# Denizantip/py-numpy-renderer

Measured on AMD Instinct MI355X. Metric: Mfrag/s (1920x1080, 200k tris + shadow volumes), higher is better.
Workload: dtype f64; 1 GPU; torus 500x200 (200k tris) + floor, 1920x1080, point light, shadow volumes (BASELINE.json configs[3] / BASELINE.md c4); faces=200002, views=8, frames_in_flight=3, parallelism=screen tiles x1 (bands)

## Files before the change

### py-numpy-renderer_amd/csrc/host_env.h

```cpp
#pragma once

namespace {

struct Env {
    bool vertex_mfma, resolve_separate, sil_cache, big_tri_reject;
    int edge_spread, tile_split, tile_order;
    int quad_walk;
    int pair_log;
    int ao_shape, dof_shape, mblur_shape, taa_shape;
    int bloom_shape;
    int tone_form, tone_grid;
    unsigned split_cost, split_quads;
    const char *cluster_cull;
};

Env read_env()
{
    static const Env once = [] {
        auto is = [](const char *name, const char *value) { const char *e = getenv(name); return e && !strcmp(e, value); };
        auto number = [](const char *name, int unset) { const char *e = getenv(name); return e ? atoi(e) : unset; };
        auto shape = [&](const char *name, const char *s0, const char *s1, const char *s2) {
            return is(name, s0) ? 0 : is(name, s1) ? 1 : is(name, s2) ? 2 : 0;
        };
        Env e = {};
// ... 9 lines not shown
        e.ao_shape = shape("MR_AO_TILE", "64x64", "32x32", "64x16");
        e.dof_shape = shape("MR_DOF_TILE", "32x32", "32x32x256", "16x16");
        e.mblur_shape = shape("MR_MBLUR_TILE", "32x32", "32x32x256", "16x16");
        e.taa_shape = shape("MR_TAA_TILE", "32x8", "64x4", "16x16");
        e.bloom_shape = shape("MR_BLOOM_TILE", "32x8", "64x4", "16x16");
        e.tone_form = is("MR_TONEMAP_HIST", "ballot") ? 1 : 0;
        e.tone_grid = std::min(std::max(number("MR_TONEMAP_GRID", (int)mr::TONE_HIST_BLOCKS), 1), (int)mr::TONE_MAX_BLOCKS);
        return e;
    }();
    Env e = once;
    e.cluster_cull = getenv("MR_CLUSTER_CULL");
    const char *sil = getenv("MR_SIL_CACHE");
    e.sil_cache = !(sil && !strcmp(sil, "0"));
    const char *rej = getenv("MR_BIG_TRI_REJECT");
    e.big_tri_reject = !(rej && !strcmp(rej, "0"));
    return e;
}

}
```

### py-numpy-renderer_amd/csrc/host_frame.h

```cpp
#pragma once

namespace {

constexpr int EVENT_RING = 512, N_MARKS = 6;

struct FrameSlot {
    hipStream_t stream = nullptr;
    int id = 0;
    DevBuf d_vout, d_vclip, d_tris, d_clips, d_status, d_count_list, d_quads, d_sil, d_counters;
    DevBuf d_bin_count, d_items[mr::BIN_CLASSES], d_work, d_tile_stats, d_hist, d_split;
    DevBuf d_z, d_winner, d_stencil, d_frame, d_out;
    DevBuf d_frame_b;
    DevBuf d_bloom;
    DevBuf d_shafts;
    DevBuf d_tone;
    int last_tone = 0;
    float last_tone_exposure = 0.f;
    MotionSlot motion;
    MotionFacesSlot motion_faces;
    LayersSlot layers;
    int last_layers = 0;
    bool last_motion = false;
    DevBuf d_stencil_x[mr::MAX_LIGHTS - 1];
    static_assert(mr::MAX_LIGHTS == MR_MAX_LIGHTS, "the ABI's light count is the kernels'");
    int last_n_lights = 1;
// ... 12 lines not shown

    mr_frame_desc last_frame = {};
    int last_n_tiles = 0;
    bool last_ordered = false;
    bool last_full = false, last_split = false;
    bool overlay_deferred = false;
    int last_ss_mode = 0;
    bool last_post = false;
    bool have_frame = false, stats_reduced = false;
    bool last_copied = false;

    void reset_caps() { bins_zeroed_for = 0; have_frame = false; }
    void release()
    {
        for (DevBuf *b : { &d_vout, &d_vclip, &d_count_list, &d_tris, &d_clips, &d_status, &d_quads, &d_sil, &d_counters,
                           &d_bin_count, &d_work, &d_tile_stats, &d_hist, &d_split, &d_z, &d_winner, &d_stencil, &d_frame, &d_frame_b, &d_bloom, &d_shafts, &d_tone, &d_out })
            b->release();
        for (DevBuf &b : d_items) b.release();
        for (DevBuf &b : d_stencil_x) b.release();
        motion.release();
        motion_faces.release();
        layers.release();
        ov.release();
        if (events_ok) {
            for (auto &set : ev_ring) for (auto &e : set) (void)hipEventDestroy(e);
            (void)hipHostFree(h_counters);
            events_ok = false;
        }
    }
    mr::Counters *ctr(uint64_t frame) const { return d_counters.as<mr::Counters>() + (frame & 1); }
    mr::Sticky *sticky() const { return reinterpret_cast<mr::Sticky *>(d_counters.as<mr::Counters>() + 2); }
// ... 335 lines not shown
        { fs->d_frame_b, p.dof || p.motion || p.taa ? kept_f * 3 * sizeof(float) : 0 },
        { fs->d_bloom, p.bloom ? bloom_pyramid(fc.width, fc.height, p.bloom_params.levels).floats * sizeof(float) : 0 },
        { fs->d_shafts, p.shafts ? 2 * shafts_level(fc.width, fc.height, p.shafts_params.levels).device_floats() * sizeof(float) : 0 },
        { fs->d_tone, p.tone ? tone_slot_bytes(tone_grid(fc.width, fc.height, p.env)) : 0 } };
    for (const auto &b : sized) HIP_TRY(b.buf.ensure(b.bytes));
    if (p.taa)
        if (int rc = grow_history(sc, fc.width, fc.height)) return rc;
    for (int k = 1; k < p.n_lights; ++k) HIP_TRY(fs->d_stencil_x[k - 1].ensure(kept * sizeof(int32_t)));
    if (int rc = ensure_cleared(fs->d_counters, 2 * sizeof(Counters) + sizeof(Sticky), fs->stream)) return rc;
    for (int c = 0; c < BIN_CLASSES; ++c) {
        const size_t bytes = nT * fs->bin_cap[c] * 4;
        if (bytes > ((size_t)48 << 30))
            return fail(MR_E_OVERFLOW, "more primitives in one 16x16 tile than the tile lists are allowed to grow to (48 GB per class)");
        HIP_TRY(fs->d_items[c].ensure(bytes));
    }
    if (!fs->events_ok) {
        for (auto &set : fs->ev_ring) for (auto &e : set) HIP_TRY(hipEventCreate(&e));
        HIP_TRY(hipHostMalloc((void **)&fs->h_counters, sizeof(Counters) + sizeof(Sticky), hipHostMallocDefault));
        fs->h_sticky = reinterpret_cast<Sticky *>(fs->h_counters + 1);
        fs->events_ok = true;
    }
    return MR_OK;
}

int grow_tile_state(FrameSlot *fs, const FramePlan &p)
{
    using namespace mr;
    HIP_TRY(fs->d_hist.ensure(p.order_bytes + (size_t)std::max(p.n_tiles, 1) + 16));
    constexpr size_t arrive_bytes = (size_t)HEAVY0_MAX * 4;
    if (int rc = ensure_cleared(fs->d_split, arrive_bytes + arrive_bytes * HEAVY_SPLIT * TILE_PX, fs->stream, arrive_bytes)) return rc;
    if (fs->bins_zeroed_for != BIN_CLASSES * p.n_tiles + 1) {
        HIP_TRY(hipMemsetAsync(fs->d_bin_count.p, 0, fs->d_bin_count.cap, fs->stream));
        HIP_TRY(hipMemsetAsync(fs->d_hist.p, 0, fs->d_hist.cap, fs->stream));
        fs->bins_zeroed_for = BIN_CLASSES * p.n_tiles + 1;
    }
    return MR_OK;
}

mr::BinArgs bin_args(const FrameSlot *fs)
{
    mr::BinArgs ba;
    ba.tris = fs->d_tris.as<mr::TriRec>(); ba.quads = fs->d_quads.as<mr::QuadRec>();
    ba.ctr = fs->ctr(fs->frames_enqueued); ba.quad_cap = fs->quad_cap;
    ba.bin_count = fs->d_bin_count.as<uint32_t>();
    for (int c = 0; c < mr::BIN_CLASSES; ++c) { ba.items[c] = fs->d_items[c].as<uint32_t>(); ba.cap[c] = fs->bin_cap[c]; }
    ba.work = fs->d_work.as<uint2>(); ba.work_cap = fs->work_cap;
    return ba;
}

int launch_setup(mr_scene *sc, FrameSlot *fs, const mr::FrameConst &fc, const FramePlan &p, const mr::FrameLights &lights)
{
    using namespace mr;
    hipStream_t stream = fs->stream;
    SetupKernArgs ska;
    ska.fc = fc; ska.bins = bin_args(fs); ska.face_blocks = p.face_blocks;
    SetupArgs &sa = ska.sa;
    sa.faces = sc->d_faces.as<int32_t>(); sa.face_flags = sc->d_face_flags.as<uint8_t>();
    sa.verts = sc->d_verts.as<double>(); sa.uv = sc->d_uv.as<float>(); sa.normals = sc->d_normals.as<float>();
    sa.vout = fs->d_vout.as<VertexOut>(); sa.vclip = fs->d_vclip.as<VertexClip>();
    sa.face_pos = sc->d_face_pos.p; sa.clusters = sc->d_clusters.as<ClusterRec>();
    sa.tris = fs->d_tris.as<TriRec>(); sa.clips = fs->d_clips.as<TriClip>();
// ... 40 lines not shown
    TileArgs &ta = tka.ta;
    ta.clips = fs->d_clips.as<TriClip>(); ta.quads = fs->d_quads.as<QuadRec>();
    ta.bin_count = fs->d_bin_count.as<uint32_t>();
    for (int c = 0; c < BIN_CLASSES; ++c) { ta.items[c] = fs->d_items[c].as<uint32_t>(); ta.cap[c] = fs->bin_cap[c]; }
    ta.tap_mask = (p.overlay && !p.taps_asked) ? fs->ov.list<uint8_t>(3) : nullptr;
    ta.zbuf = p.keep ? fs->d_z.as<double>() : nullptr;
    ta.winner = p.keep ? fs->d_winner.as<int32_t>() : nullptr;
    ta.stencil = p.keep ? fs->d_stencil.as<int32_t>() : nullptr;
    ta.tile_stats = fs->d_tile_stats.as<uint32_t>();
    ta.ctr = fs->ctr(fs->frames_enqueued); ta.next_ctr = fs->ctr(fs->frames_enqueued + 1); ta.sticky = fs->sticky();
    ta.order = p.ordered ? fs->d_hist.as<uint32_t>() : nullptr;
    ta.tile_class = reinterpret_cast<uint8_t *>(fs->d_hist.p) + p.order_bytes;
    ta.split_arrive = fs->d_split.as<uint32_t>(); ta.split_sten = fs->d_split.as<int32_t>() + HEAVY0_MAX;
    ta.split_cost = p.split_cost; ta.split_quads = p.split_quads; ta.split_max = p.split_max;
    ta.quad_walk = (uint32_t)p.env.quad_walk;
    ta.pair_log = (uint32_t)fc.n_faces <= PAIR_LOG_MAX_FACE ? (uint32_t)p.env.pair_log : 0u;
    ShadeArgs &sh = tka.sh;
    sh.tris = fs->d_tris.as<TriRec>(); sh.face_pos = sc->d_face_pos.p; sh.face_attr = sc->d_face_attr.as<FaceAttr>();
    sh.materials = sc->d_materials.as<Material>();
    sh.sky = sc->sky_size > 0 ? sc->d_sky.as<uint8_t>() : nullptr;
    sh.gamma_lut = sc->d_gamma.as<float>(); sh.out = d_out;
    sh.frame = (fc.flags & MR_FRAME_KEEP_FLOAT) ? fs->d_frame.as<float>() : nullptr;
    tka.ml.lights.n = 1;
    if (p.ml) tka.ml.lights = lights;
    for (int k = 1; p.ml && k < MAX_LIGHTS; ++k) tka.ml.stencil[k - 1] = p.keep && k < p.n_lights ? fs->d_stencil_x[k - 1].as<int32_t>() : nullptr;
    if (p.n_tiles <= 0) {
        HIP_TRY(hipMemsetAsync(ta.next_ctr, 0, sizeof(Counters), fs->stream));
        return MR_OK;
    }
    static const struct { void (*kernel)(const TileKernArgs); int front; } choice[2][6] = {
// ... 225 lines not shown
```

### py-numpy-renderer_amd/csrc/kernels_bin.h

```cpp
#pragma once

#include "rast_math.h"
#include "tri_reject.h"

namespace mr {

struct TileSpan { int tx0, tx1, ty0, ty1; };

__device__ __forceinline__ int tile_row_frame(const FrameConst &fc, int l) { return fc.tile_y0 + l * fc.tile_step; }

__device__ __forceinline__ bool tile_span(const FrameConst &fc, int x0, int x1, int y0, int y1, TileSpan &s)
{
    y0 = max(y0, fc.band_y0);
    y1 = min(y1, fc.band_y1);
    if (x0 >= x1 || y0 >= y1) return false;
    s.tx0 = x0 / TILE_W;            s.tx1 = (x1 - 1) / TILE_W + 1;
    const int g0 = y0 / TILE_H - fc.tile_y0, g1 = (y1 - 1) / TILE_H - fc.tile_y0;
    if (g1 < 0) return false;
    const int st = fc.tile_step;
    s.ty0 = g0 <= 0 ? 0 : (g0 + st - 1) / st;
    s.ty1 = min(g1 / st + 1, fc.tiles_y);
    return s.ty0 < s.ty1;
}

// ... 14 lines not shown
    bool out = o0 || o1 || o2 || (n > 3 && o3);
    for (int i = 4; i < n && !out; ++i) out = outside(q.e[i]);
    return !out;
}

struct BinArgs {
    const TriRec *tris;
    const QuadRec *quads;
    Counters *ctr;
    uint32_t quad_cap;
    uint32_t *bin_count;
    uint32_t *items[BIN_CLASSES];
    uint32_t cap[BIN_CLASSES];
    uint2 *work;
    uint32_t work_cap;
};

constexpr int TILE_STATS = 5;
constexpr int TILE_REC = 12;
constexpr int QUAD_BATCH = 64;
constexpr int BIN_SMALL = 4;
constexpr uint32_t WORK_QUAD = 0x80000000u;
constexpr int ORDER_CLASSES = 8;
constexpr int ORDER_HEAD = 4;

struct PrimBox { int x0, x1, y0, y1; };

__device__ __forceinline__ int pair_class(const FrameConst &fc, bool is_quad, bool clip, const PrimBox &pb, int tx, int ty)
{
    if (is_quad) return 2;
// ... 156 lines not shown
        if (!tile_span(fc, pb.x0, pb.x1, pb.y0, pb.y1, sp)) continue;
        const int bw = sp.tx1 - sp.tx0, total = bw * (sp.ty1 - sp.ty0);
        const int j = (int)item.y * WAVE + lane;
        if (j >= total) continue;
        const int tx = sp.tx0 + j % bw, ty = sp.ty0 + j / bw;
        bool touches;
        if (is_quad) {
            touches = quad_touches_tile(a.quads[id], tx, tile_row_frame(fc, ty));
        } else {
            touches = !big_tri_reject || tri_touches_tile(a.tris[id], tx * TILE_W, tile_row_frame(fc, ty) * TILE_H);
            if (fc.flags & MR_FRAME_COUNTERS) {
                const unsigned long long out = __ballot(!touches);
                if (out && lane == __ffsll((long long)out) - 1) atomicAdd(&a.ctr->pad0[7], (unsigned int)__popcll(out));
            }
        }
        if (touches) bin_emit(fc, a, pair_class(fc, is_quad, clip, pb, tx, ty), id, tx, ty);
    }
}

__device__ void order_tiles_block(const uint8_t *__restrict__ cls, uint32_t *__restrict__ order, int n_tiles)
{
    constexpr int NT = 256, NW = NT / WAVE, NC = ORDER_CLASSES + 1, FIELD = 12, LOW = 5;
    __shared__ uint32_t s_cnt[NC][NT];
    __shared__ uint32_t s_tot[NC];
    const int tid = threadIdx.x, lane = tid & (WAVE - 1), wv = tid / WAVE;
    const int per = ((n_tiles + NT - 1) / NT + 3) & ~3;
    const int t0 = tid * per, nwords = per >> 2;
    const uint32_t *__restrict__ words = reinterpret_cast<const uint32_t *>(cls);
    auto fetch = [&](int i) -> uint32_t {
        const int t = t0 + 4 * i;
        uint32_t v = t < n_tiles ? words[t >> 2] : 0xffffffffu;
// ... 76 lines not shown
```

### py-numpy-renderer_amd/csrc/kernels_tile.h

```cpp
#pragma once

#include "kernels_bin.h"
#include "kernels_shade.h"
#include "rast_resolve.h"

namespace mr {

__device__ __forceinline__ unsigned long long z_key(double z)
{
    const unsigned long long b = (unsigned long long)__double_as_longlong(z);
    return (b >> 63) ? ~b : (b | 0x8000000000000000ull);
}
__device__ __forceinline__ double z_unkey(unsigned long long k)
{
    const unsigned long long b = (k >> 63) ? (k & 0x7fffffffffffffffull) : ~k;
    return __longlong_as_double((long long)b);
}

template <bool MAYBE_SINGLE>
struct PairMath {
    double a0, a1, p0, p1, q0, q1, k0, k1, k2;
    float d00, d01, d11, inv_den;
    bool sbox, sz;
    __device__ __forceinline__ explicit PairMath(const TriRec &t)
// ... 132 lines not shown
    double nx, ny, nz, d;
    int16_t x0, x1, y0, y1;
    int32_t n, is_front, edge;
    uint32_t pad[3];
};
static_assert(sizeof(QuadHead) == 64, "QuadHead mirrors QuadRec's header");

enum : uint32_t { QUAD_WALK_AUTO = 0, QUAD_WALK_STRIPS = 1, QUAD_WALK_SPANS = 2 };
#ifndef MR_SPAN_MIN_EDGES
#define MR_SPAN_MIN_EDGES 1
#endif
#ifndef MR_SPAN_MIN_QUADS
#define MR_SPAN_MIN_QUADS 6
#endif

__device__ __forceinline__ bool quad_depth_pass(double q_nx, double q_ny, double nzq, double q_d, double a0, double b0,
                                                double dpx, double dpy, double zbest, bool rh, bool in,
                                                double f_plus_n, double f_minus_n, double two_nf)
{
    const double t = (q_nx * dpx + q_ny * dpy) + q_d;
    const double tf = t * f_minus_n;
    const double den = a0 + tf;
    const double prod = zbest * den;
    const double e = prod - b0;
    const bool zinf = fabs(zbest) == INFINITY;
    bool pass = zinf ? (rh ? zbest > 0 : zbest < 0) : (rh ? ((e > 0) == (den > 0)) : ((e < 0) == (den > 0)));
    const bool clear = zinf || fabs(e) > 1e-9 * (fabs(prod) + fabs(b0));
    const bool unsure = in && !(clear && fabs(den) > 2e-4 * (fabs(a0) + fabs(tf)));
    if (__ballot(unsure)) {
        if (unsure) {
            const double z = two_nf / (f_plus_n - (-t / nzq) * f_minus_n);
            pass = rh ? (zbest >= z) : (zbest <= z);
        }
    }
    return pass;
}

constexpr int MAT_LDS = 8;
static_assert(sizeof(Material) % 8 == 0 && MAT_LDS * sizeof(Material) / 8 <= TILE_PX, "material staging");

#ifndef MR_CLASS_SCALE
#define MR_CLASS_SCALE 100
#endif
__device__ __forceinline__ int tile_class(uint32_t cost)
{
    const uint32_t c = cost * 100u / (uint32_t)MR_CLASS_SCALE;
    return c >= 500u ? 1 : c >= 350u ? 2 : c >= 250u ? 3 : c >= 170u ? 4 : c >= 110u ? 5 : c >= 70u ? 6 : c >= 40u ? 7 : 8;
}
static_assert(ORDER_CLASSES == 8, "tile_class");
#ifndef MR_HEAVY0_MAX
#define MR_HEAVY0_MAX 128
// ... 22 lines not shown
    uint32_t cap[BIN_CLASSES];
    uint32_t pair_log;
    const uint8_t *tap_mask;
    double *zbuf;
    int32_t *winner, *stencil;
    uint32_t *tile_stats;
    Counters *ctr, *next_ctr;
    Sticky *sticky;
    int32_t *split_sten;
    uint32_t *split_arrive;
    const uint32_t *order;
    uint8_t *tile_class;
    uint32_t split_cost, split_quads;
    uint32_t split_max;
    uint32_t quad_walk;
};

struct TileLights {
    FrameLights lights;
    int32_t *stencil[MAX_LIGHTS - 1];
};
struct TileKernArgs { FrameConst fc; TileArgs ta; ShadeArgs sh; TileLights ml; };

template <bool SPLIT, bool SS, bool ML, bool FULL>
__device__ __forceinline__ void tile_body()
{
    static_assert(!(SPLIT && ML), "frames with several lights do not split their heavy tiles");
    __shared__ unsigned long long s_key[TILE_PX];
    __shared__ int s_win[TILE_PX];
    __shared__ unsigned int s_cnt[TILE_STATS];
    __shared__ uint4 s_quad[QUAD_BATCH * QUAD_STAGE_U4];
    __shared__ uint32_t s_id[QUAD_BATCH];
    __shared__ float s_gamma[GAMMA_LUT_SIZE];
    __shared__ unsigned long long s_mat[MAT_LDS * sizeof(Material) / 8];

    const int tid = threadIdx.x, lane = tid & (WAVE - 1);
    const int lp = tid;
    auto stamp = []() -> unsigned long long { return FULL ? __builtin_amdgcn_s_memrealtime() : 0ull; };

    int tile = 0, part = 0, n_parts = 1, entry = 0, n_tiles, ltr, gx, gy;
    bool rh, counters, live, mat_lds, taps;
    uint32_t n_small_raw, n_big_raw, n_quad_raw, n_small, n_big, n_quad, cost;
    unsigned long long t_start;
    {
        const TileKernArgs &ka = kernargs<TileKernArgs>();
        const FrameConst &fc = ka.fc;
        const TileArgs &ta = ka.ta;
        const ShadeArgs &sh = ka.sh;
        n_tiles = fc.tiles_x * fc.tiles_y;
// ... 83 lines not shown
                o[0] = (uint8_t)fc.background_u8; o[1] = (uint8_t)(fc.background_u8 >> 8); o[2] = (uint8_t)(fc.background_u8 >> 16);
            }
            if (tid == 0) {
                uint32_t *rec = ta.tile_stats + (size_t)tile * TILE_REC;
                for (int k = 0; k < TILE_REC; ++k) rec[k] = 0;
                rec[7] = n_quad_raw;
                rec[8] = rec[10] = rec[11] = (uint32_t)t_start;
                rec[9] = (uint32_t)stamp();
                ta.bin_count[2 * n_tiles + tile] = 0;
                ta.tile_class[tile] = (uint8_t)ORDER_CLASSES;
            }
            return;
        }
        if (FULL && tid == 0) ta.tile_stats[(size_t)tile * TILE_REC + 8] = (uint32_t)t_start;
        if (FULL && tid < TILE_STATS) s_cnt[tid] = 0;
        s_gamma[tid] = sh.gamma_lut[tid];
        if (tid == 0) s_gamma[GAMMA_LUT_SIZE - 1] = sh.gamma_lut[GAMMA_LUT_SIZE - 1];
        mat_lds = fc.n_materials <= MAT_LDS;
        if (mat_lds && tid < fc.n_materials * (int)(sizeof(Material) / 8))
            s_mat[tid] = reinterpret_cast<const unsigned long long *>(sh.materials)[tid];
    }
    auto my_pixel = [&](int &px, int &py) {
        int l = lp;
        asm volatile("" : "+v"(l));
        px = gx + (l & (TILE_W - 1)); py = gy + l / TILE_W;
    };

    double zbest = rh ? INFINITY : -INFINITY;
    int best = -1;
    {
// ... 109 lines not shown
                if (lane == 0 && a) atomicAdd(&ta.ctr->pad0[5], a);
                if (lane == 0 && b) atomicAdd(&ta.ctr->pad0[6], b);
            }
            __syncthreads();
            best = s_win[lp];
            zbest = z_unkey(kfinal);
        }
        if (has_no_depth) big_pairs(true);
    }
    const bool covered = live && best >= 0;
    const unsigned long long t_raster = stamp();

    int sten = 0;
    int sten_x[MAX_LIGHTS - 1] = { 0, 0, 0 };
    unsigned int qfrags = 0, qupd = 0;
    if (n_quad && (counters || __syncthreads_or(covered))) {
        const TileKernArgs &ka = kernargs<TileKernArgs>();
        const FrameConst &fc = ka.fc;
        const TileArgs &ta = ka.ta;
        const uint32_t *__restrict__ quad_items = ta.items[2] + (size_t)tile * ta.cap[2];
        const QuadRec *__restrict__ quads = ta.quads;
        const double f_plus_n = fc.f_plus_n, f_minus_n = fc.f_minus_n, two_nf = fc.two_nf;
        double zlim = rh ? -INFINITY : INFINITY, zhard = rh ? INFINITY : -INFINITY;
        if (covered) zlim = zhard = zbest;
#pragma unroll
        for (int off = WAVE / 2; off; off >>= 1) {
            const double o = __shfl_xor(zlim, off), h = __shfl_xor(zhard, off);
            zlim = rh ? fmax(zlim, o) : fmin(zlim, o);
            zhard = rh ? fmin(zhard, h) : fmax(zhard, h);
        }
        if (!FULL) {
            zlim = __hiloint2double(__builtin_amdgcn_readfirstlane(__double2hiint(zlim)), __builtin_amdgcn_readfirstlane(__double2loint(zlim)));
            zhard = __hiloint2double(__builtin_amdgcn_readfirstlane(__double2hiint(zhard)), __builtin_amdgcn_readfirstlane(__double2loint(zhard)));
        }
        if (!ML && ta.quad_walk != QUAD_WALK_STRIPS) {
            if (!n_small) s_key[lp] = z_key(zbest);
            s_win[lp] = 0;
        }
        const uint32_t q_begin = SPLIT ? (uint32_t)((unsigned long long)part * n_quad / n_parts) : 0u,
                       q_end = SPLIT ? (uint32_t)((unsigned long long)(part + 1) * n_quad / n_parts) : n_quad;
        for (uint32_t qbase = q_begin; qbase < q_end; qbase += QUAD_BATCH) {
            const int n = (int)min((uint32_t)QUAD_BATCH, q_end - qbase);
            if (qbase != q_begin) __syncthreads();
            for (int i = tid; i < n * QUAD_STAGE_U4; i += TILE_PX) {
                const int q = i / QUAD_STAGE_U4, piece = i - q * QUAD_STAGE_U4;
                const uint32_t id = quad_items[qbase + q];
                const QuadRec *src = quads + id;
                uint4 val = reinterpret_cast<const uint4 *>(src)[piece];
                if (piece == 3) {
                    const double a0 = f_plus_n * src->nz, b0 = two_nf * src->nz;
                    val = make_uint4((uint32_t)__double2loint(a0), (uint32_t)__double2hiint(a0),
                                     (uint32_t)__double2loint(b0), (uint32_t)__double2hiint(b0));
                } else if (piece >= 5 && (piece & 1) && !src->is_front) {
                    val.y ^= 0x80000000u; val.w ^= 0x80000000u;
                } else if (ML && piece == 2) {
                    val.w |= src->light << 1;
                }
                s_quad[i] = val;
                if (piece == 0) s_id[q] = id;
            }
            __syncthreads();

            bool q_reject = lane >= n;
            bool q_finite = true;
            int emask = 0;
            if (!q_reject) {
                const QuadHead &h = *reinterpret_cast<const QuadHead *>(s_quad + lane * QUAD_STAGE_U4);
                const QuadEdge *e = reinterpret_cast<const QuadEdge *>(s_quad + lane * QUAD_STAGE_U4 + 4);
                const double xa = (double)gx, xb = (double)(gx + TILE_W - 1);
                const double ya = (double)(gy + (tid / WAVE) * (WAVE / TILE_W)), yb = ya + (double)(WAVE / TILE_W - 1);
                if (h.n > 4) emask |= 16;
#pragma unroll
                for (int i = 0; i < 4; ++i) {
                    if (i < 3 || h.n > 3) {
// ... 1 lines not shown
                        const double py0 = (ya - e[i].sy) * e[i].ex, py1 = (yb - e[i].sy) * e[i].ex;
                        const double c00 = px0 - py0, c10 = px1 - py0, c01 = px0 - py1, c11 = px1 - py1;
                        const bool any = c00 > 0 || c10 > 0 || c01 > 0 || c11 > 0;
                        const bool all = c00 > 0 && c10 > 0 && c01 > 0 && c11 > 0;
                        q_reject = q_reject || !any;
                        if (!ML) q_finite = q_finite && fabs(px0) + fabs(px1) + fabs(py0) + fabs(py1) < INFINITY;
                        if (!all) emask |= 1 << i;
                    }
                }
            }
            bool q_allpass = false;
            if (!q_reject) {
                const QuadHead &h = *reinterpret_cast<const QuadHead *>(s_quad + lane * QUAD_STAGE_U4);
                const double xa = (double)gx, xb = (double)(gx + TILE_W - 1);
                const double ya = (double)(gy + (tid / WAVE) * (WAVE / TILE_W)), yb = ya + (double)(WAVE / TILE_W - 1);
                const double t00 = (h.nx * xa + h.ny * ya) + h.d, t10 = (h.nx * xb + h.ny * ya) + h.d;
                const double t01 = (h.nx * xa + h.ny * yb) + h.d, t11 = (h.nx * xb + h.ny * yb) + h.d;
                const double tmin = fmin(fmin(t00, t10), fmin(t01, t11)), tmax = fmax(fmax(t00, t10), fmax(t01, t11));
                const double inz = approx_rcp(h.nz);
                const double za = -tmin * inz, zb = -tmax * inz;
                const double slack = 1e-12 * fmax(fabs(za), fabs(zb)) +
                                     1e-15 * ((fabs(h.nx) * xb + fabs(h.ny) * yb) + fabs(h.d)) * fabs(inz);
                const double zs_lo = fmin(za, zb) - slack, zs_hi = fmax(za, zb) + slack;
                const double den_lo = f_plus_n - zs_hi * f_minus_n, den_hi = f_plus_n - zs_lo * f_minus_n;
                double fpn = f_plus_n, tnf = two_nf;
                if (!ML) asm volatile("" : "+v"(fpn), "+v"(tnf));
                const bool sane = two_nf > 0 && f_minus_n > 0 && den_lo > 1e-9 * fpn && h.nz != 0 &&
                                  fabs(inz) < 1e300 && den_hi < 1e300;
                const double lo = tnf * (1.0 - 1e-12), hi = tnf * (1.0 + 1e-12);
                const bool none = rh ? lo > zlim * den_hi : hi < zlim * den_lo;
                const bool all = rh ? hi <= zhard * den_lo : lo >= zhard * den_hi;
                if (sane && !counters && none) q_reject = true;
                q_allpass = sane && all;
            }
            unsigned long long todo = __ballot(!q_reject);
            const unsigned long long allpass = __ballot(q_allpass);

            const uint32_t quad_walk = ML ? (uint32_t)QUAD_WALK_STRIPS : kernargs<TileKernArgs>().ta.quad_walk;
            if (!ML && quad_walk != QUAD_WALK_STRIPS) {
                const bool span_ok = !q_reject && q_finite && !(emask & 16);
                unsigned long long smask = __ballot(span_ok && (quad_walk == QUAD_WALK_SPANS || __popc(emask & 15) >= MR_SPAN_MIN_EDGES));
                if (quad_walk == QUAD_WALK_AUTO && __popcll(smask) < MR_SPAN_MIN_QUADS) smask = 0;
                todo &= ~smask;
                if (smask) {
                    const int cnt = __popcll(smask);
                    const int rank = (int)__builtin_amdgcn_mbcnt_hi((uint32_t)(smask >> 32), __builtin_amdgcn_mbcnt_lo((uint32_t)smask, 0u));
                    int ln = lane;
                    if (!FULL) asm volatile("" : "+v"(ln));
// ... 112 lines not shown
                                       f_plus_n, f_minus_n, two_nf);
                }
                pass = pass && in;
                if (FULL) qupd += (unsigned int)__popcll(__ballot(pass));
                if (ML) {
                    const int lt = __builtin_amdgcn_readfirstlane((int)(hb.w >> 1)), d = pass ? (front ? 1 : -1) : 0;
                    if (lt == 0) sten += d;
                    else if (lt == 1) sten_x[0] += d;
                    else if (lt == 2) sten_x[1] += d;
                    else sten_x[2] += d;
                } else {
                sten += pass ? (front ? 1 : -1) : 0;
                }
            }
        }
        if (!ML && kernargs<TileKernArgs>().ta.quad_walk != QUAD_WALK_STRIPS) {
            __syncthreads();
            sten += s_win[lp];
        }
    }

    if (SPLIT && n_parts > 1) {
        __shared__ uint32_t s_ticket;
        const TileArgs &ta = kernargs<TileKernArgs>().ta;
        int32_t *mine = ta.split_sten + ((size_t)entry * HEAVY_SPLIT + part) * TILE_PX;
        int l = lp;
        if (!FULL) asm volatile("" : "+v"(l));
        mine[l] = sten;
        asm volatile("s_waitcnt vmcnt(0)" ::: "memory");
        __syncthreads();
        if (tid == 0) {
            __builtin_amdgcn_fence(__ATOMIC_RELEASE, "agent");
            asm volatile("s_waitcnt vmcnt(0)" ::: "memory");
            s_ticket = atomicAdd(&ta.split_arrive[entry], 1u);
        }
        __syncthreads();
        if (s_ticket != (uint32_t)(n_parts - 1)) return;
        if (tid == 0) {
            __builtin_amdgcn_fence(__ATOMIC_ACQUIRE, "agent");
            asm volatile("s_waitcnt vmcnt(0)" ::: "memory");
            ta.split_arrive[entry] = 0;
        }
        __syncthreads();
        for (int k = 0; k < n_parts; ++k)
            if (k != part) sten += ta.split_sten[((size_t)entry * HEAVY_SPLIT + k) * TILE_PX + l];
    }
    const unsigned long long t_quads = stamp();

    const bool lit = (int16_t)sten == 0;
    unsigned int n_lit = lit ? 1u : 0u;
    const bool fused_ss = SS && !(kernargs<TileKernArgs>().fc.ss_mode & SS_SEPARATE);
    if (fused_ss) __syncthreads();
    unsigned int lit_mask = lit ? 1u : 0u;
    if (ML) {
        const TileKernArgs &ka = kernargs<TileKernArgs>();
        const int n_lights = min(max(ka.ml.lights.n, 1), MAX_LIGHTS);
#pragma unroll
        for (int k = 1; k < MAX_LIGHTS; ++k)
            if (k < n_lights && (int16_t)sten_x[k - 1] == 0) lit_mask |= 1u << k;
        if (live && ka.ta.zbuf && taps) {
// ... 89 lines not shown
            if (lane == 0 && v) atomicAdd(&s_cnt[4], v);
        }
        if (lane == 0) {
            if (cov) atomicAdd(&s_cnt[3], (unsigned int)__popcll(cov));
            if (!ML && litm) atomicAdd(&s_cnt[4], (unsigned int)__popcll(litm));
            if (qfrags) atomicAdd(&s_cnt[1], qfrags);
            if (qupd) atomicAdd(&s_cnt[2], qupd);
        }
    }
    if (FULL) __syncthreads();
    const TileArgs &ta = kernargs<TileKernArgs>().ta;
    uint32_t *rec = ta.tile_stats + (size_t)tile * TILE_REC;
    if (FULL && tid < TILE_STATS) rec[tid] = s_cnt[tid];
    if (tid == 0) {
        rec[5] = n_small_raw; rec[6] = n_big_raw; rec[7] = n_quad_raw;
        if (!FULL) rec[8] = 0;
        rec[9] = (uint32_t)stamp();
        rec[10] = (uint32_t)t_raster; rec[11] = (uint32_t)t_quads;
        if (n_small_raw > ta.cap[0]) { atomicOr(&ta.ctr->overflow, 1u); atomicMax(&ta.ctr->max_list[0], n_small_raw); }
        if (n_big_raw > ta.cap[1]) { atomicOr(&ta.ctr->overflow, 2u); atomicMax(&ta.ctr->max_list[1], n_big_raw); }
        if (n_quad_raw > ta.cap[2]) { atomicOr(&ta.ctr->overflow, 4u); atomicMax(&ta.ctr->max_list[2], n_quad_raw); }
    }
    if (tid < BIN_CLASSES) ta.bin_count[tid * n_tiles + tile] = 0;
    if (tid == 0) {
        int cls = tile_class(cost);
        if (SPLIT) cls = (cost >= ta.split_cost && n_quad_raw >= ta.split_quads) ? 1 : cls < 2 ? 2 : cls;
        ta.tile_class[tile] = (uint8_t)cls;
    }
}

template <bool SPLIT, bool SS, bool ML>
// ... 80 lines not shown
```

Measured before the change: 40220 Mfrag/s.

## Precompute per-tile quad depth bounds at binning and cull quads per tile

During binning, each shadow-volume quad's conservative denominator bound for the whole 16x16 tile is computed and stored as a float next to its tile list entry. In the tile kernel's single-light, non-counter path, the tile's farthest depth is reduced into shared memory. Quads whose bound proves they cannot affect any pixel are then dropped per wave, and survivors are compacted with ballot and permute before being staged into LDS. This is meant to skip staging and per-pixel stencil work for occluded shadow quads. The cost is an extra bound buffer, extra binning arithmetic, another block reduction and sync, and reliance on the float rounding used for the bound.

```diff
diff --git a/py-numpy-renderer_amd/csrc/host_env.h b/py-numpy-renderer_amd/csrc/host_env.h
--- a/py-numpy-renderer_amd/csrc/host_env.h
+++ b/py-numpy-renderer_amd/csrc/host_env.h
@@ -5,6 +5,7 @@
 struct Env {
     bool vertex_mfma, resolve_separate, sil_cache, big_tri_reject;
     int edge_spread, tile_split, tile_order;
+    int quad_tile_cull;
     int quad_walk;
     int pair_log;
     int ao_shape, dof_shape, mblur_shape, taa_shape;
@@ -47,6 +48,8 @@
     e.sil_cache = !(sil && !strcmp(sil, "0"));
     const char *rej = getenv("MR_BIG_TRI_REJECT");
     e.big_tri_reject = !(rej && !strcmp(rej, "0"));
+    const char *cull = getenv("MR_QUAD_TILE_CULL");
+    e.quad_tile_cull = !cull ? 1 : !strcmp(cull, "0") ? 0 : !strcmp(cull, "count") ? 3 : !strcmp(cull, "count0") ? 2 : 1;
     return e;
 }
 
diff --git a/py-numpy-renderer_amd/csrc/host_frame.h b/py-numpy-renderer_amd/csrc/host_frame.h
--- a/py-numpy-renderer_amd/csrc/host_frame.h
+++ b/py-numpy-renderer_amd/csrc/host_frame.h
@@ -8,7 +8,7 @@
     hipStream_t stream = nullptr;
     int id = 0;
     DevBuf d_vout, d_vclip, d_tris, d_clips, d_status, d_count_list, d_quads, d_sil, d_counters;
-    DevBuf d_bin_count, d_items[mr::BIN_CLASSES], d_work, d_tile_stats, d_hist, d_split;
+    DevBuf d_bin_count, d_items[mr::BIN_CLASSES], d_quad_bound, d_work, d_tile_stats, d_hist, d_split;
     DevBuf d_z, d_winner, d_stencil, d_frame, d_out;
     DevBuf d_frame_b;
     DevBuf d_bloom;
@@ -51,7 +51,7 @@
     void release()
     {
         for (DevBuf *b : { &d_vout, &d_vclip, &d_count_list, &d_tris, &d_clips, &d_status, &d_quads, &d_sil, &d_counters,
-                           &d_bin_count, &d_work, &d_tile_stats, &d_hist, &d_split, &d_z, &d_winner, &d_stencil, &d_frame, &d_frame_b, &d_bloom, &d_shafts, &d_tone, &d_out })
+                           &d_bin_count, &d_quad_bound, &d_work, &d_tile_stats, &d_hist, &d_split, &d_z, &d_winner, &d_stencil, &d_frame, &d_frame_b, &d_bloom, &d_shafts, &d_tone, &d_out })
             b->release();
         for (DevBuf &b : d_items) b.release();
         for (DevBuf &b : d_stencil_x) b.release();
@@ -417,6 +417,8 @@
             return fail(MR_E_OVERFLOW, "more primitives in one 16x16 tile than the tile lists are allowed to grow to (48 GB per class)");
         HIP_TRY(fs->d_items[c].ensure(bytes));
     }
+    HIP_TRY(fs->d_quad_bound.ensure(nT * fs->bin_cap[2] * sizeof(float)));
+
     if (!fs->events_ok) {
         for (auto &set : fs->ev_ring) for (auto &e : set) HIP_TRY(hipEventCreate(&e));
         HIP_TRY(hipHostMalloc((void **)&fs->h_counters, sizeof(Counters) + sizeof(Sticky), hipHostMallocDefault));
@@ -431,7 +433,7 @@
     using namespace mr;
     HIP_TRY(fs->d_hist.ensure(p.order_bytes + (size_t)std::max(p.n_tiles, 1) + 16));
     constexpr size_t arrive_bytes = (size_t)HEAVY0_MAX * 4;
-    if (int rc = ensure_cleared(fs->d_split, arrive_bytes + arrive_bytes * HEAVY_SPLIT * TILE_PX, fs->stream, arrive_bytes)) return rc;
+    if (int rc = ensure_cleared(fs->d_split, arrive_bytes + arrive_bytes * HEAVY_SPLIT * TILE_PX + arrive_bytes * HEAVY_SPLIT, fs->stream, arrive_bytes)) return rc;
     if (fs->bins_zeroed_for != BIN_CLASSES * p.n_tiles + 1) {
         HIP_TRY(hipMemsetAsync(fs->d_bin_count.p, 0, fs->d_bin_count.cap, fs->stream));
         HIP_TRY(hipMemsetAsync(fs->d_hist.p, 0, fs->d_hist.cap, fs->stream));
@@ -448,6 +450,7 @@
     ba.bin_count = fs->d_bin_count.as<uint32_t>();
     for (int c = 0; c < mr::BIN_CLASSES; ++c) { ba.items[c] = fs->d_items[c].as<uint32_t>(); ba.cap[c] = fs->bin_cap[c]; }
     ba.work = fs->d_work.as<uint2>(); ba.work_cap = fs->work_cap;
+    ba.quad_bound = fs->d_quad_bound.as<float>();
     return ba;
 }
 
@@ -518,6 +521,7 @@
     ta.split_arrive = fs->d_split.as<uint32_t>(); ta.split_sten = fs->d_split.as<int32_t>() + HEAVY0_MAX;
     ta.split_cost = p.split_cost; ta.split_quads = p.split_quads; ta.split_max = p.split_max;
     ta.quad_walk = (uint32_t)p.env.quad_walk;
+    ta.quad_bound = fs->d_quad_bound.as<float>(); ta.quad_cull = (uint32_t)p.env.quad_tile_cull;
     ta.pair_log = (uint32_t)fc.n_faces <= PAIR_LOG_MAX_FACE ? (uint32_t)p.env.pair_log : 0u;
     ShadeArgs &sh = tka.sh;
     sh.tris = fs->d_tris.as<TriRec>(); sh.face_pos = sc->d_face_pos.p; sh.face_attr = sc->d_face_attr.as<FaceAttr>();
diff --git a/py-numpy-renderer_amd/csrc/kernels_bin.h b/py-numpy-renderer_amd/csrc/kernels_bin.h
--- a/py-numpy-renderer_amd/csrc/kernels_bin.h
+++ b/py-numpy-renderer_amd/csrc/kernels_bin.h
@@ -2,6 +2,7 @@
 
 #include "rast_math.h"
 #include "tri_reject.h"
+#include "quad_reject.h"
 
 namespace mr {
 
@@ -52,6 +53,7 @@
     uint32_t cap[BIN_CLASSES];
     uint2 *work;
     uint32_t work_cap;
+    float *quad_bound;
 };
 
 constexpr int TILE_STATS = 5;
@@ -238,7 +240,18 @@
                 if (out && lane == __ffsll((long long)out) - 1) atomicAdd(&a.ctr->pad0[7], (unsigned int)__popcll(out));
             }
         }
-        if (touches) bin_emit(fc, a, pair_class(fc, is_quad, clip, pb, tx, ty), id, tx, ty);
+        if (touches && is_quad) {
+            const QuadRec &q = a.quads[id];
+            const uint32_t tile = (uint32_t)ty * fc.tiles_x + tx;
+            const uint32_t pos = atomicAdd(&a.bin_count[2u * (uint32_t)(fc.tiles_x * fc.tiles_y) + tile], 1u);
+            if (pos < a.cap[2]) {
+                a.items[2][(size_t)tile * a.cap[2] + pos] = id;
+                a.quad_bound[(size_t)tile * a.cap[2] + pos] = quad_tile_bound(q.nx, q.ny, q.nz, q.d, tx * TILE_W, tile_row_frame(fc, ty) * TILE_H,
+                                                                             TILE_W, TILE_H, fc.f_plus_n, fc.f_minus_n, fc.two_nf, fc.system == 1);
+            }
+        } else if (touches) {
+            bin_emit(fc, a, pair_class(fc, false, clip, pb, tx, ty), id, tx, ty);
+        }
     }
 }
 
diff --git a/py-numpy-renderer_amd/csrc/kernels_tile.h b/py-numpy-renderer_amd/csrc/kernels_tile.h
--- a/py-numpy-renderer_amd/csrc/kernels_tile.h
+++ b/py-numpy-renderer_amd/csrc/kernels_tile.h
@@ -170,27 +170,6 @@
 #define MR_SPAN_MIN_QUADS 6
 #endif
 
-__device__ __forceinline__ bool quad_depth_pass(double q_nx, double q_ny, double nzq, double q_d, double a0, double b0,
-                                                double dpx, double dpy, double zbest, bool rh, bool in,
-                                                double f_plus_n, double f_minus_n, double two_nf)
-{
-    const double t = (q_nx * dpx + q_ny * dpy) + q_d;
-    const double tf = t * f_minus_n;
-    const double den = a0 + tf;
-    const double prod = zbest * den;
-    const double e = prod - b0;
-    const bool zinf = fabs(zbest) == INFINITY;
-    bool pass = zinf ? (rh ? zbest > 0 : zbest < 0) : (rh ? ((e > 0) == (den > 0)) : ((e < 0) == (den > 0)));
-    const bool clear = zinf || fabs(e) > 1e-9 * (fabs(prod) + fabs(b0));
-    const bool unsure = in && !(clear && fabs(den) > 2e-4 * (fabs(a0) + fabs(tf)));
-    if (__ballot(unsure)) {
-        if (unsure) {
-            const double z = two_nf / (f_plus_n - (-t / nzq) * f_minus_n);
-            pass = rh ? (zbest >= z) : (zbest <= z);
-        }
-    }
-    return pass;
-}
 
 constexpr int MAT_LDS = 8;
 static_assert(sizeof(Material) % 8 == 0 && MAT_LDS * sizeof(Material) / 8 <= TILE_PX, "material staging");
@@ -243,6 +222,8 @@
     uint32_t split_cost, split_quads;
     uint32_t split_max;
     uint32_t quad_walk;
+    const float *quad_bound;
+    uint32_t quad_cull;
 };
 
 struct TileLights {
@@ -262,6 +243,8 @@
     __shared__ uint32_t s_id[QUAD_BATCH];
     __shared__ float s_gamma[GAMMA_LUT_SIZE];
     __shared__ unsigned long long s_mat[MAT_LDS * sizeof(Material) / 8];
+    constexpr bool CULL = !FULL && !ML;
+    __shared__ unsigned long long s_zt;
 
     const int tid = threadIdx.x, lane = tid & (WAVE - 1);
     const int lp = tid;
@@ -375,6 +358,7 @@
         }
         if (FULL && tid == 0) ta.tile_stats[(size_t)tile * TILE_REC + 8] = (uint32_t)t_start;
         if (FULL && tid < TILE_STATS) s_cnt[tid] = 0;
+        if (CULL && tid == 0) s_zt = rh ? 0ull : ~0ull;
         s_gamma[tid] = sh.gamma_lut[tid];
         if (tid == 0) s_gamma[GAMMA_LUT_SIZE - 1] = sh.gamma_lut[GAMMA_LUT_SIZE - 1];
         mat_lds = fc.n_materials <= MAT_LDS;
@@ -514,7 +498,19 @@
     int sten = 0;
     int sten_x[MAX_LIGHTS - 1] = { 0, 0, 0 };
     unsigned int qfrags = 0, qupd = 0;
-    if (n_quad && (counters || __syncthreads_or(covered))) {
+    unsigned int q_kept = 0;
+    int zt_seen = 0;
+    if (CULL && n_quad) {
+        if (__ballot(covered)) {
+            double zw = covered ? zbest : (rh ? -INFINITY : INFINITY);
+#pragma unroll
+            for (int off = WAVE / 2; off; off >>= 1) { const double o = __shfl_xor(zw, off); zw = rh ? fmax(zw, o) : fmin(zw, o); }
+            if (lane == 0) { if (rh) atomicMax(&s_zt, z_key(zw)); else atomicMin(&s_zt, z_key(zw)); }
+        }
+        __syncthreads();
+        zt_seen = __builtin_amdgcn_readfirstlane(s_zt != (rh ? 0ull : ~0ull) ? 1 : 0);
+    }
+    if (n_quad && (CULL ? zt_seen != 0 : (counters || __syncthreads_or(covered)))) {
         const TileKernArgs &ka = kernargs<TileKernArgs>();
         const FrameConst &fc = ka.fc;
         const TileArgs &ta = ka.ta;
@@ -533,31 +529,77 @@
             zlim = __hiloint2double(__builtin_amdgcn_readfirstlane(__double2hiint(zlim)), __builtin_amdgcn_readfirstlane(__double2loint(zlim)));
             zhard = __hiloint2double(__builtin_amdgcn_readfirstlane(__double2hiint(zhard)), __builtin_amdgcn_readfirstlane(__double2loint(zhard)));
         }
-        if (!ML && ta.quad_walk != QUAD_WALK_STRIPS) {
+        auto span_words = [&]() {
+            if (ta.quad_walk != QUAD_WALK_STRIPS) {
+                double zb = zbest;
+                asm volatile("" : "+v"(zb));
+                if (!n_small) s_key[lp] = z_key(zb);
+                s_win[lp] = 0;
+            }
+        };
+        if (!CULL && !ML && ta.quad_walk != QUAD_WALK_STRIPS) {
             if (!n_small) s_key[lp] = z_key(zbest);
             s_win[lp] = 0;
         }
         const uint32_t q_begin = SPLIT ? (uint32_t)((unsigned long long)part * n_quad / n_parts) : 0u,
                        q_end = SPLIT ? (uint32_t)((unsigned long long)(part + 1) * n_quad / n_parts) : n_quad;
         for (uint32_t qbase = q_begin; qbase < q_end; qbase += QUAD_BATCH) {
-            const int n = (int)min((uint32_t)QUAD_BATCH, q_end - qbase);
-            if (qbase != q_begin) __syncthreads();
-            for (int i = tid; i < n * QUAD_STAGE_U4; i += TILE_PX) {
-                const int q = i / QUAD_STAGE_U4, piece = i - q * QUAD_STAGE_U4;
-                const uint32_t id = quad_items[qbase + q];
-                const QuadRec *src = quads + id;
-                uint4 val = reinterpret_cast<const uint4 *>(src)[piece];
-                if (piece == 3) {
-                    const double a0 = f_plus_n * src->nz, b0 = two_nf * src->nz;
-                    val = make_uint4((uint32_t)__double2loint(a0), (uint32_t)__double2hiint(a0),
-                                     (uint32_t)__double2loint(b0), (uint32_t)__double2hiint(b0));
-                } else if (piece >= 5 && (piece & 1) && !src->is_front) {
-                    val.y ^= 0x80000000u; val.w ^= 0x80000000u;
-                } else if (ML && piece == 2) {
-                    val.w |= src->light << 1;
-                }
-                s_quad[i] = val;
-                if (piece == 0) s_id[q] = id;
+            int n = (int)min((uint32_t)QUAD_BATCH, q_end - qbase);
+            if (CULL) {
+                bool keep = lane < n;
+                uint32_t my_id = 0;
+                if (keep) {
+                    my_id = quad_items[qbase + lane];
+                    if (ta.quad_cull & 1u) {
+                        double tnf = two_nf;
+                        asm volatile("" : "+v"(tnf));
+                        keep = !quad_tile_none(ta.quad_bound[(size_t)tile * ta.cap[2] + qbase + lane], z_unkey(s_zt), tnf, rh);
+                    }
+                }
+                const unsigned long long km = __ballot(keep);
+                n = __popcll(km);
+                if (!n) continue;
+                const int rank = (int)__builtin_amdgcn_mbcnt_hi((uint32_t)(km >> 32), __builtin_amdgcn_mbcnt_lo((uint32_t)km, 0u));
+                const int ids = __builtin_amdgcn_ds_permute((keep ? rank : n + (lane - rank)) << 2, (int)my_id);
+                if (q_kept) __syncthreads();
+                else span_words();
+                q_kept += (unsigned int)n;
+                for (int i0 = 0; i0 < n * QUAD_STAGE_U4; i0 += TILE_PX) {
+                    const int i = i0 + tid, q = i / QUAD_STAGE_U4, piece = i - q * QUAD_STAGE_U4;
+                    const uint32_t id = (uint32_t)__builtin_amdgcn_ds_bpermute(q << 2, ids);
+                    if (i < n * QUAD_STAGE_U4) {
+                        const QuadRec *src = quads + id;
+                        uint4 val = reinterpret_cast<const uint4 *>(src)[piece];
+                        if (piece == 3) {
+                            const double a0 = f_plus_n * src->nz, b0 = two_nf * src->nz;
+                            val = make_uint4((uint32_t)__double2loint(a0), (uint32_t)__double2hiint(a0),
+                                             (uint32_t)__double2loint(b0), (uint32_t)__double2hiint(b0));
+                        } else if (piece >= 5 && (piece & 1) && !src->is_front) {
+                            val.y ^= 0x80000000u; val.w ^= 0x80000000u;
+                        }
+                        s_quad[i] = val;
+                        if (piece == 0) s_id[q] = id;
+                    }
+                }
+            } else {
+                if (qbase != q_begin) __syncthreads();
+                for (int i = tid; i < n * QUAD_STAGE_U4; i += TILE_PX) {
+                    const int q = i / QUAD_STAGE_U4, piece = i - q * QUAD_STAGE_U4;
+                    const uint32_t id = quad_items[qbase + q];
+                    const QuadRec *src = quads + id;
+                    uint4 val = reinterpret_cast<const uint4 *>(src)[piece];
+                    if (piece == 3) {
+                        const double a0 = f_plus_n * src->nz, b0 = two_nf * src->nz;
+                        val = make_uint4((uint32_t)__double2loint(a0), (uint32_t)__double2hiint(a0),
+                                         (uint32_t)__double2loint(b0), (uint32_t)__double2hiint(b0));
+                    } else if (piece >= 5 && (piece & 1) && !src->is_front) {
+                        val.y ^= 0x80000000u; val.w ^= 0x80000000u;
+                    } else if (ML && piece == 2) {
+                        val.w |= src->light << 1;
+                    }
+                    s_quad[i] = val;
+                    if (piece == 0) s_id[q] = id;
+                }
             }
             __syncthreads();
 
@@ -589,24 +631,13 @@
                 const QuadHead &h = *reinterpret_cast<const QuadHead *>(s_quad + lane * QUAD_STAGE_U4);
                 const double xa = (double)gx, xb = (double)(gx + TILE_W - 1);
                 const double ya = (double)(gy + (tid / WAVE) * (WAVE / TILE_W)), yb = ya + (double)(WAVE / TILE_W - 1);
-                const double t00 = (h.nx * xa + h.ny * ya) + h.d, t10 = (h.nx * xb + h.ny * ya) + h.d;
-                const double t01 = (h.nx * xa + h.ny * yb) + h.d, t11 = (h.nx * xb + h.ny * yb) + h.d;
-                const double tmin = fmin(fmin(t00, t10), fmin(t01, t11)), tmax = fmax(fmax(t00, t10), fmax(t01, t11));
-                const double inz = approx_rcp(h.nz);
-                const double za = -tmin * inz, zb = -tmax * inz;
-                const double slack = 1e-12 * fmax(fabs(za), fabs(zb)) +
-                                     1e-15 * ((fabs(h.nx) * xb + fabs(h.ny) * yb) + fabs(h.d)) * fabs(inz);
-                const double zs_lo = fmin(za, zb) - slack, zs_hi = fmax(za, zb) + slack;
-                const double den_lo = f_plus_n - zs_hi * f_minus_n, den_hi = f_plus_n - zs_lo * f_minus_n;
+                const QuadRectBounds b = quad_rect_bounds(h.nx, h.ny, h.nz, h.d, xa, xb, ya, yb, f_plus_n, f_minus_n);
                 double fpn = f_plus_n, tnf = two_nf;
                 if (!ML) asm volatile("" : "+v"(fpn), "+v"(tnf));
-                const bool sane = two_nf > 0 && f_minus_n > 0 && den_lo > 1e-9 * fpn && h.nz != 0 &&
-                                  fabs(inz) < 1e300 && den_hi < 1e300;
-                const double lo = tnf * (1.0 - 1e-12), hi = tnf * (1.0 + 1e-12);
-                const bool none = rh ? lo > zlim * den_hi : hi < zlim * den_lo;
-                const bool all = rh ? hi <= zhard * den_lo : lo >= zhard * den_hi;
-                if (sane && !counters && none) q_reject = true;
-                q_allpass = sane && all;
+                const bool sane = quad_rect_sane(b, h.nz, f_minus_n, two_nf, fpn);
+                const QuadRectVerdict v = quad_rect_verdict(b, tnf, zlim, zhard, rh);
+                if (sane && !counters && v.none) q_reject = true;
+                q_allpass = sane && v.all;
             }
             unsigned long long todo = __ballot(!q_reject);
             const unsigned long long allpass = __ballot(q_allpass);
@@ -749,7 +780,7 @@
                 }
             }
         }
-        if (!ML && kernargs<TileKernArgs>().ta.quad_walk != QUAD_WALK_STRIPS) {
+        if (!ML && (!CULL || q_kept) && kernargs<TileKernArgs>().ta.quad_walk != QUAD_WALK_STRIPS) {
             __syncthreads();
             sten += s_win[lp];
         }
@@ -762,6 +793,8 @@
         int l = lp;
         if (!FULL) asm volatile("" : "+v"(l));
         mine[l] = sten;
+        uint32_t *kept = reinterpret_cast<uint32_t *>(ta.split_sten + (size_t)HEAVY0_MAX * HEAVY_SPLIT * TILE_PX) + (size_t)entry * HEAVY_SPLIT;
+        if (CULL && tid == 0) kept[part] = q_kept;
         asm volatile("s_waitcnt vmcnt(0)" ::: "memory");
         __syncthreads();
         if (tid == 0) {
@@ -779,6 +812,9 @@
         __syncthreads();
         for (int k = 0; k < n_parts; ++k)
             if (k != part) sten += ta.split_sten[((size_t)entry * HEAVY_SPLIT + k) * TILE_PX + l];
+        if (CULL)
+            for (int k = 0; k < n_parts; ++k)
+                if (k != part) q_kept += __atomic_load_n(&kept[k], __ATOMIC_RELAXED);
     }
     const unsigned long long t_quads = stamp();
 
@@ -898,7 +934,7 @@
     if (FULL && tid < TILE_STATS) rec[tid] = s_cnt[tid];
     if (tid == 0) {
         rec[5] = n_small_raw; rec[6] = n_big_raw; rec[7] = n_quad_raw;
-        if (!FULL) rec[8] = 0;
+        if (!FULL) rec[8] = (ta.quad_cull & 2u) ? q_kept : 0u;
         rec[9] = (uint32_t)stamp();
         rec[10] = (uint32_t)t_raster; rec[11] = (uint32_t)t_quads;
         if (n_small_raw > ta.cap[0]) { atomicOr(&ta.ctr->overflow, 1u); atomicMax(&ta.ctr->max_list[0], n_small_raw); }
diff --git a/py-numpy-renderer_amd/csrc/quad_reject.h b/py-numpy-renderer_amd/csrc/quad_reject.h
--- /dev/null
+++ b/py-numpy-renderer_amd/csrc/quad_reject.h
@@ -0,0 +1,115 @@
+#pragma once
+
+#include <math.h>
+#include <stdint.h>
+#include <string.h>
+
+#if defined(__HIPCC__)
+#define MR_QUAD_FN __device__ __forceinline__
+#define MR_QUAD_ANY(x) __ballot(x)
+#else
+#define MR_QUAD_FN inline
+#define MR_QUAD_ANY(x) (x)
+#endif
+
+namespace mr {
+
+#if !defined(__HIPCC__)
+#ifndef MR_QUAD_HOST_RCP
+#define MR_QUAD_HOST_RCP(x) (1.0 / (x))
+#endif
+inline double approx_rcp(double x) { return MR_QUAD_HOST_RCP(x); }
+#endif
+
+MR_QUAD_FN bool quad_depth_pass(double q_nx, double q_ny, double nzq, double q_d, double a0, double b0,
+                                double dpx, double dpy, double zbest, bool rh, bool in,
+                                double f_plus_n, double f_minus_n, double two_nf)
+{
+    const double t = (q_nx * dpx + q_ny * dpy) + q_d;
+    const double tf = t * f_minus_n;
+    const double den = a0 + tf;
+    const double prod = zbest * den;
+    const double e = prod - b0;
+    const bool zinf = fabs(zbest) == INFINITY;
+    bool pass = zinf ? (rh ? zbest > 0 : zbest < 0) : (rh ? ((e > 0) == (den > 0)) : ((e < 0) == (den > 0)));
+    const bool clear = zinf || fabs(e) > 1e-9 * (fabs(prod) + fabs(b0));
+    const bool unsure = in && !(clear && fabs(den) > 2e-4 * (fabs(a0) + fabs(tf)));
+    if (MR_QUAD_ANY(unsure)) {
+        if (unsure) {
+            const double z = two_nf / (f_plus_n - (-t / nzq) * f_minus_n);
+            pass = rh ? (zbest >= z) : (zbest <= z);
+        }
+    }
+    return pass;
+}
+
+struct QuadRectBounds { double den_lo, den_hi, inz; };
+MR_QUAD_FN QuadRectBounds quad_rect_bounds(double nx, double ny, double nz, double d, double xa, double xb, double ya, double yb,
+                                           double f_plus_n, double f_minus_n)
+{
+    const double t00 = (nx * xa + ny * ya) + d, t10 = (nx * xb + ny * ya) + d;
+    const double t01 = (nx * xa + ny * yb) + d, t11 = (nx * xb + ny * yb) + d;
+    const double tmin = fmin(fmin(t00, t10), fmin(t01, t11)), tmax = fmax(fmax(t00, t10), fmax(t01, t11));
+    const double inz = approx_rcp(nz);
+    const double za = -tmin * inz, zb = -tmax * inz;
+    const double slack = 1e-12 * fmax(fabs(za), fabs(zb)) +
+                         1e-15 * ((fabs(nx) * xb + fabs(ny) * yb) + fabs(d)) * fabs(inz);
+    const double zs_lo = fmin(za, zb) - slack, zs_hi = fmax(za, zb) + slack;
+    QuadRectBounds b;
+    b.den_lo = f_plus_n - zs_hi * f_minus_n; b.den_hi = f_plus_n - zs_lo * f_minus_n; b.inz = inz;
+    return b;
+}
+MR_QUAD_FN bool quad_rect_sane(const QuadRectBounds &b, double nz, double f_minus_n, double two_nf, double fpn)
+{
+    return two_nf > 0 && f_minus_n > 0 && b.den_lo > 1e-9 * fpn && nz != 0 &&
+           fabs(b.inz) < 1e300 && b.den_hi < 1e300;
+}
+
+struct QuadRectVerdict { bool none, all; };
+MR_QUAD_FN QuadRectVerdict quad_rect_verdict(const QuadRectBounds &b, double tnf, double zlim, double zhard, bool rh)
+{
+    const double lo = tnf * (1.0 - 1e-12), hi = tnf * (1.0 + 1e-12);
+    QuadRectVerdict v;
+    v.none = rh ? lo > zlim * b.den_hi : hi < zlim * b.den_lo;
+    v.all = rh ? hi <= zhard * b.den_lo : lo >= zhard * b.den_hi;
+    return v;
+}
+
+
+MR_QUAD_FN float quad_bound_f32(double x, bool away)
+{
+    const double m = fabs(x);
+    if (!(m >= 0x1p-100 && m <= 0x1p100)) return NAN;
+    float f = (float)m;
+    uint32_t bits;
+    memcpy(&bits, &f, 4);
+    if (away ? (double)f < m : (double)f > m) bits += away ? 1u : 0xffffffffu;
+    memcpy(&f, &bits, 4);
+    return x < 0 ? -f : f;
+}
+
+MR_QUAD_FN bool quad_rect_sane_neg(const QuadRectBounds &b, double nz, double f_minus_n, double two_nf, double fpn)
+{
+    return two_nf > 0 && f_minus_n > 0 && b.den_hi < -1e-9 * fpn && nz != 0 &&
+           fabs(b.inz) < 1e300 && b.den_lo > -1e300;
+}
+
+MR_QUAD_FN float quad_tile_bound(double nx, double ny, double nz, double d, int gx, int gy, int tile_w, int tile_h,
+                                 double f_plus_n, double f_minus_n, double two_nf, bool rh)
+{
+    const QuadRectBounds b = quad_rect_bounds(nx, ny, nz, d, (double)gx, (double)(gx + tile_w - 1), (double)gy, (double)(gy + tile_h - 1),
+                                              f_plus_n, f_minus_n);
+    if (quad_rect_sane(b, nz, f_minus_n, two_nf, f_plus_n)) return quad_bound_f32(rh ? b.den_hi : b.den_lo, rh);
+    if (quad_rect_sane_neg(b, nz, f_minus_n, two_nf, f_plus_n)) return quad_bound_f32(rh ? b.den_hi : b.den_lo, !rh);
+    return NAN;
+}
+
+MR_QUAD_FN bool quad_tile_none(float bound, double zt, double tnf, bool rh)
+{
+    const double lo = tnf * (1.0 - 1e-12), hi = tnf * (1.0 + 1e-12);
+    const double prod = zt * (double)bound;
+    if (bound < 0) return rh ? prod > hi : prod < lo;
+    return rh ? lo > prod : hi < prod;
+}
+
+}
```

New measurement: 42340 Mfrag/s, median of 6. +5.3%, better.
